# Jeffrey-Ede/AI-CV-Automation-Elect-Micr

Measured on AMD Instinct MI355X. Metric: megapixels/sec restored (512x512x1 bs=32), higher is better.
Workload: dtype bf16x3 (split-bf16 MFMA inputs, fp32 accumulate and activations)

## Files before the change

### ai-cv-automation-elect-micr_amd/_lib.py

```python
from __future__ import annotations

import ctypes as C
import os

PKG_DIR = os.path.dirname(os.path.abspath(__file__))
LIB_PATH = os.environ.get("EMD_LIB_PATH") or os.path.join(PKG_DIR, "libemdenoise.so")

EMD_OK = 0
EMD_K_SYMMETRIC = 1

_c_float_p = C.c_void_p

class PackJob(C.Structure):
    _fields_ = [("w", C.c_void_p), ("hi", C.c_void_p), ("lo", C.c_void_p), ("tap_sel", C.c_ulonglong), ("total", C.c_long),
                ("first_block", C.c_long), ("n_blocks", C.c_long), ("ntaps", C.c_int), ("cin", C.c_int), ("cout", C.c_int),
                ("cout_major", C.c_int), ("cpad", C.c_int), ("pad_", C.c_int)]


class KFusedJob(C.Structure):
    _fields_ = [("theta", C.c_void_p), ("adam_m", C.c_void_p), ("adam_v", C.c_void_p), ("step", C.c_void_p),
                ("params_out", C.c_void_p), ("losses", C.c_void_p), ("width", C.c_int), ("depth", C.c_int)]


SIGNATURES = {
# ... 188 lines not shown
    "emd_conv3x3_cout1_wgrad_f32": (C.c_int, [_c_float_p, C.c_int, _c_float_p, _c_float_p] + [C.c_int] * 4 + [C.c_void_p]),
    "emd_conv3x3_cout1_bwd_data_f32": (C.c_int, [_c_float_p, _c_float_p, _c_float_p, C.c_int] + [C.c_int] * 4 + [C.c_void_p]),
    "emd_resize_bilinear_bwd_f32": (C.c_int, [_c_float_p, C.c_int, _c_float_p, C.c_int] + [C.c_int] * 6 + [C.c_void_p]),
    "emd_avgpool2x2_bwd_f32": (C.c_int, [_c_float_p, C.c_int, _c_float_p, C.c_int] + [C.c_int] * 4 + [C.c_void_p]),
    "emd_axpy_f32": (C.c_int, [_c_float_p, C.c_int, _c_float_p, C.c_int, C.c_long, C.c_int, C.c_float, C.c_void_p]),
    "emd_denoise_loss_workspace_bytes": (C.c_size_t, []),
    "emd_denoise_loss_f32": (C.c_int, [_c_float_p, _c_float_p, C.c_long, C.c_float, _c_float_p, _c_float_p, C.c_void_p,
                                       C.c_void_p]),
    "emd_nesterov_step_f32": (C.c_int, [_c_float_p, _c_float_p, _c_float_p, C.c_long, C.c_float, C.c_float, C.c_float,
                                        C.c_void_p]),
    "emd_dw3x3_reflect_f32": (C.c_int, [_c_float_p, C.c_int, _c_float_p, _c_float_p, C.c_int] + [C.c_int] * 5 + [C.c_void_p]),
    "emd_cin1_k7_reflect_f32": (C.c_int, [_c_float_p] * 5 + [C.c_int] * 6 + [C.c_void_p]),
    "emd_conv3x3_cout1_reflect_f32": (C.c_int, [_c_float_p, C.c_int, _c_float_p, C.c_float, _c_float_p] + [C.c_int] * 4 +
                                      [C.c_void_p]),
    "emd_instnorm_tanh_f32": (C.c_int, [_c_float_p] * 4 + [C.c_int, C.c_long, C.c_float, C.c_void_p]),
    "emd_sep3x3_fused_reflect_f32": (C.c_int, [_c_float_p, C.c_int, _c_float_p, C.c_void_p, C.c_void_p, _c_float_p, _c_float_p,
                                               _c_float_p, _c_float_p, _c_float_p, C.c_int, _c_float_p, C.c_int, C.c_int,
                                               C.c_int, C.c_int, C.c_int, C.c_int, C.c_int, C.c_int, C.c_void_p]),
    "emd_dw3x3_reflect_gen_f32": (C.c_int, [_c_float_p, C.c_int, _c_float_p, _c_float_p, C.c_int, _c_float_p, _c_float_p] +
                                  [C.c_int] * 6 + [C.c_void_p]),
    "emd_sep3x3_fused_gen_f32": (C.c_int, [_c_float_p, C.c_int, _c_float_p, _c_float_p, C.c_int, _c_float_p, C.c_void_p,
                                           C.c_void_p, _c_float_p, _c_float_p, _c_float_p, _c_float_p, _c_float_p, C.c_int,
                                           _c_float_p, C.c_int] + [C.c_int] * 8 + [C.c_void_p]),
    "emd_fc_rows_f32": (C.c_int, [_c_float_p, C.c_int, _c_float_p, C.c_float, _c_float_p, C.c_int, C.c_int, C.c_void_p]),
    "emd_max3_sigmoid_f32": (C.c_int, [_c_float_p] * 4 + [C.c_int, C.c_void_p]),
    "emd_gan_head_f32": (C.c_int, [_c_float_p, C.c_float, C.c_int, C.c_float, _c_float_p, _c_float_p, C.c_void_p]),
    "emd_fc_row_bwd_f32": (C.c_int, [_c_float_p] * 6 + [C.c_int, C.c_void_p]),
    "emd_bcast_rows_f32": (C.c_int, [_c_float_p, _c_float_p, C.c_int, C.c_long, C.c_int, C.c_float, C.c_void_p]),
    "emd_sumsq_workspace_bytes": (C.c_size_t, []),
    "emd_sumsq_f32": (C.c_int, [_c_float_p, C.c_long, C.c_float, _c_float_p, C.c_void_p, C.c_void_p]),
    "emd_adam_step_f32": (C.c_int, [_c_float_p] * 4 + [C.c_long] + [C.c_float] * 5 + [_c_float_p, C.c_float, C.c_void_p]),
    "emd_dw3x3_reflect_wgrad_f32": (C.c_int, [_c_float_p, C.c_int, _c_float_p, C.c_int, _c_float_p] + [C.c_int] * 5 + [C.c_void_p]),
    "emd_dw3x3_reflect_bwd_data_f32": (C.c_int, [_c_float_p, C.c_int, _c_float_p, _c_float_p, C.c_int] + [C.c_int] * 5 + [C.c_void_p]),
    "emd_conv3x3_cout1_reflect_wgrad_f32": (C.c_int, [_c_float_p, C.c_int, _c_float_p, _c_float_p] + [C.c_int] * 4 + [C.c_void_p]),
    "emd_conv3x3_cout1_reflect_bwd_data_f32": (C.c_int, [_c_float_p, _c_float_p, _c_float_p, C.c_int] + [C.c_int] * 4 + [C.c_void_p]),
    "emd_dw7_c1_reflect_f32": (C.c_int, [_c_float_p] * 3 + [C.c_int] * 3 + [C.c_void_p]),
    "emd_dw7_c1_reflect_wgrad_f32": (C.c_int, [_c_float_p] * 3 + [C.c_int] * 3 + [C.c_void_p]),
    "emd_tanh_bwd_f32": (C.c_int, [_c_float_p] * 3 + [C.c_long, C.c_void_p]),
    "emd_l1_feature_f32": (C.c_int, [_c_float_p, _c_float_p, C.c_long, C.c_float, _c_float_p, C.c_int, _c_float_p, C.c_void_p]),
    "emd_crop_scatter_f32": (C.c_int, [_c_float_p, C.c_int, _c_float_p] + [C.c_int] * 4 + [C.c_void_p]),
    "emd_crop_scatter_dev_f32": (C.c_int, [_c_float_p, C.c_int, _c_float_p, C.c_void_p, C.c_int, C.c_int, C.c_void_p]),
    "emd_adam_step_dev_f32": (C.c_int, [_c_float_p] * 4 + [C.c_long, _c_float_p] + [C.c_float] * 4 + [_c_float_p, C.c_float, C.c_void_p]),
    "emd_bn_infer_fold2_f32": (C.c_int, [_c_float_p] * 8 + [C.c_float, C.c_int] + [_c_float_p] * 6 + [C.c_void_p]),
    "emd_bn_infer_grads_f32": (C.c_int, [_c_float_p] * 4 + [C.c_int] + [_c_float_p] * 4 + [C.c_void_p]),
    "emd_sep3x3_gemm_supported": (C.c_int, [C.c_int] * 4),
    "emd_sep3x3_gemm_f32": (C.c_int, [_c_float_p, C.c_int, _c_float_p, C.c_void_p, C.c_void_p, _c_float_p, _c_float_p, _c_float_p, _c_float_p,
# ... 177 lines not shown
```

### ai-cv-automation-elect-micr_amd/csrc/graph_exec.hip

```cpp
#include <cmath>
#include <cstdlib>
#include <cstring>
#include <map>
#include <string>
#include <vector>

#include "graph_common.hpp"

namespace {

constexpr int F0 = 64, F1 = 128, F2 = 256, F3 = 728, F4 = 728, AF = 728, AOUT = 256, NEXTRA = 11;
constexpr double BN_EPS = 1e-3;

enum Kind { SEP, CONV, DECONV, BNONLY };

struct LayerDecl {
    std::string key;
    Kind kind;
    int cin, cout, k = 1, stride = 1, rate = 1;
    std::string wname = "weights", bname = "biases";
    std::string scope;
    std::vector<std::string> bn;
    std::string extra_bn;
};
// ... 387 lines not shown
        }
        T4 cur[2] = {part(x, 0), part(x, 1)}, oh[2] = {part(out, 0), part(out, 1)};
        for (int blk = -1; blk < NEXTRA; ++blk)
            for (int h = 0; h < 2; ++h) {
                ar = &sub[h];
                st = dry ? st0 : g->side[h];
                middle_block(blk, &cur[h], &oh[h]);
            }
        ar = ar0;
        st = st0;
        if (!dry) {
            for (int h = 0; h < 2; ++h)
                if (hipEventRecord(g->join[h], g->side[h]) != hipSuccess || hipStreamWaitEvent(st0, g->join[h], 0) != hipSuccess)
                    call(emd::fail(EMD_E_LAUNCH, "emd_graph_run: stream join failed"));
        }
        for (int h = 0; h < 2; ++h) ar->release(mem[h]);
        return out;
    }

    void forward(const float* xin, float* yout, int B, int S) {
        const int S2 = S / 2, S4 = S / 4, S16 = S / 16;
        auto& P = g->P;
        T4 cnn0_last;
        if (emd_sep3x3_fused_supported(S, S, F0, F0, 1, 1)) {
            T4 d4 = E(B, S, S, 4);
            cnn0_last = E(B, S, S, F0);
            if (live()) {
                const LayerParams &pc = P["cnn0"], &pl = P["cnn0_last"];
                call(emd_cin1_f32(xin, pc.w9, g->unit4, g->zero4, d4.ptr(), d4.ld, B, S, S, 4, 1, 0, st));
                call(emd_sep3x3_fused_gen_f32(d4.ptr(), d4.ld, pc.a, pc.shift, EMD_ACT_RELU6, pl.dw, pl.pw.hi, pl.pw.lo, pl.scale, pl.shift, nullptr,
                                              nullptr, nullptr, 0, cnn0_last.ptr(), cnn0_last.ld, B, S, S, F0, F0, EMD_ACT_RELU6, EMD_PREC_BF16X3, 0, st));
            }
            free(d4);
        } else {
            T4 cnn0 = E(B, S, S, F0);
            if (live()) call(emd_cin1_f32(xin, P["cnn0"].w9, P["cnn0"].a, P["cnn0"].shift, cnn0.ptr(), cnn0.ld, B, S, S, F0, 1, 1, st));
            cnn0_last = sep("cnn0_last", cnn0, nullptr, nullptr);
            free(cnn0);
        }
        T4 concat1 = E(B, S2, S2, F2 + F1);
        T4 c1s = concat1.slice(F2, F1);
        T4 cnn0_strided;
        const LayerParams& ps = P["cnn0_strided"];
        if (ps.d.stride == 2 && ps.d.rate == 1 && emd_sep3x3_fused_supported(S, S, ps.d.cin, ps.d.cout, 2, 1) &&
            emd_sep3x3_fused_s2_genres_supported(S, S, ps.d.cin, ps.d.cout)) {
            cnn0_strided = c1s;
            if (live())
// ... 310 lines not shown
```

### ai-cv-automation-elect-micr_amd/csrc/sep_fused.hip

```cpp
#include <cstdlib>

#include "sep_params.hpp"

using namespace emd;

namespace {

__device__ __attribute__((aligned(16))) float g_zero_px[4096];

inline int sep_nt() { return (g_knobs.nt_mask >> 1) & 1; }
inline int sep_xcd() { return g_knobs.sep_xcd; }

template <int BN, int PASSES, bool GEN, int TH = 8, bool DUAL = false, bool WRES = false>
__global__ __launch_bounds__(256, 2) void sep_fused_kernel(const SepParams p) {
    constexpr int TW = 16, BM = TH * TW, BK = 32;
    constexpr int PH = TH + 2, PW = TW + 2, NPX = PH * PW;
    constexpr int PLD = 40;
    constexpr int LDK = BK + 8;
    constexpr int WN = BN / 64, WM = 4 / WN;
    constexpr int TM = BM / WM / 32, TN = BN / WN / 32;
    constexpr int NPL = PASSES == 3 ? 2 : 1;
    constexpr int P_PASSES = (NPX * 8 + 255) / 256;
    constexpr int W_PASSES = BN / 64;
    constexpr int NPT = BM / 32;
// ... 338 lines not shown
#pragma unroll 4
                for (int r = er; r < BM; r += ROWS_PER_PASS)
                    put(r, finish(*reinterpret_cast<const f32x4*>(&stage[r][ncol])));
            }
        }
        __syncthreads();
        SEP_STAMP(6)
#pragma unroll
        for (int i = 0; i < TM; ++i)
#pragma unroll
            for (int j = 0; j < TN; ++j)
#pragma unroll
                for (int e = 0; e < 16; ++e) acc[i][j][e] = 0.f;
        x0 += TW;
    }
    if (p.stamps && tid == 0) {
        long long* o = p.stamps + ((long)(blockIdx.z * gridDim.y + blockIdx.y) * gridDim.x + blockIdx.x) * 8;
#pragma unroll
        for (int i = 0; i < 8; ++i) o[i] = ph[i];
    }
#undef SEP_STAMP
}


int tiles_per_workgroup(int tiles_w, long wgs1) {
    const int force = g_knobs.sep_tpw;
    int tpw = 1;
    for (int t = 8; t >= 2; t >>= 1)
        if (tiles_w % t == 0 && wgs1 / t >= 2048) { tpw = t; break; }
    if (force > 0 && tiles_w % force == 0) tpw = force;
    return tpw;
}

int launch_wres(const SepParams& p, int B, hipStream_t st) {
    SepParams q = p;
    const int tiles_w = p.W / 16;
    q.tpw = tiles_per_workgroup(tiles_w, (long)tiles_w * (p.H / 8) * B);
    q.stamps = g_knobs.sep_stamps;
    const dim3 grid(tiles_w / q.tpw, p.H / 8, B);
    q.nt = sep_nt();
    q.xcd = sep_xcd() && ((long)grid.x * grid.y * grid.z) % 8 == 0;
    if (p.gen_a) hipLaunchKernelGGL((sep_fused_kernel<64, 3, true, 8, false, true>), grid, dim3(256), 0, st, q);
    else hipLaunchKernelGGL((sep_fused_kernel<64, 3, false, 8, false, true>), grid, dim3(256), 0, st, q);
    return emd::check_launch("sep_fused_kernel<resident W>");
}

template <int BN>
int launch(const SepParams& p, int B, int passes, hipStream_t st) {
    if constexpr (BN == 64) {
        const int wres = g_knobs.sep_wres;
        if (wres && p.Cin <= 64 && passes == 3) return launch_wres(p, B, st);
    }
    SepParams q = p;
    const int tiles_w = p.W / 16;
    q.tpw = tiles_per_workgroup(tiles_w, (long)tiles_w * (p.H / 8) * B);
    q.stamps = g_knobs.sep_stamps;
    const dim3 grid(tiles_w / q.tpw, p.H / 8, B);
    q.nt = sep_nt();
    q.xcd = sep_xcd() && ((long)grid.x * grid.y * grid.z) % 8 == 0;
    if (p.gen_a) {
        if (passes == 3)
            hipLaunchKernelGGL((sep_fused_kernel<BN, 3, true>), grid, dim3(256), 0, st, q);
        else
            hipLaunchKernelGGL((sep_fused_kernel<BN, 1, true>), grid, dim3(256), 0, st, q);
    } else if (passes == 3)
        hipLaunchKernelGGL((sep_fused_kernel<BN, 3, false>), grid, dim3(256), 0, st, q);
    else
// ... 213 lines not shown
    return sep_fused_entry(x, ldx, dw, whi, wlo, scale1, shift1, scale2, shift2, res, ldres, static_cast<float*>(y), ldy, B, H, W, Cin,
                           Cout, act, 3, 0, stream, nullptr, nullptr, 0, 1);
}

extern "C" int emd_sep3x3_fused_reflect_f32(const float* x, int ldx, const float* dw, const uint16_t* whi,
                                            const uint16_t* wlo, const float* scale1, const float* shift1,
                                            const float* scale2, const float* shift2, const float* res, int ldres,
                                            float* y, int ldy, int B, int H, int W, int Cin, int Cout, int act,
                                            int precision, emd_stream_t stream) {
    return sep_fused_entry(x, ldx, dw, whi, wlo, scale1, shift1, scale2, shift2, res, ldres, y, ldy, B, H, W, Cin, Cout, act,
                           precision, 1, stream);
}

extern "C" int emd_sep3x3_fused_gen_f32(const float* d, int ldd, const float* gen_a, const float* gen_t, int gen_act,
                                        const float* dw, const uint16_t* whi, const uint16_t* wlo, const float* scale1,
                                        const float* shift1, const float* scale2, const float* shift2, const float* res,
                                        int ldres, float* y, int ldy, int B, int H, int W, int Cin, int Cout, int act,
                                        int precision, int reflect, emd_stream_t stream) {
    EMD_REQUIRE(gen_a && gen_t, EMD_E_INVALID, "emd_sep3x3_fused_gen_f32: null gen_a / gen_t");
    return sep_fused_entry(d, ldd, dw, whi, wlo, scale1, shift1, scale2, shift2, res, ldres, y, ldy, B, H, W, Cin, Cout, act,
                           precision, reflect, stream, gen_a, gen_t, gen_act);
}

extern "C" void emd_debug_sep_stamps(void* buf) { g_knobs.sep_stamps = static_cast<long long*>(buf); }

extern "C" int emd_sep3x3_dual_supported(int H, int W, int Cin, int Cout, int Cout2) {
    const bool wide = Cout > 64 || Cout2 > 64;
    return H % (wide ? 4 : 8) == 0 && W % 16 == 0 && Cin % 32 == 0 && Cin >= 32 && Cin <= 4096 && Cout % 4 == 0 && Cout2 % 4 == 0 &&
           Cout >= 4 && Cout2 >= 4 && Cout <= 128 && Cout2 <= 128;
}

extern "C" int emd_sep3x3_dual_preferred(int H, int W, int Cin, int Cout, int Cout2) {
    if (!emd_sep3x3_dual_supported(H, W, Cin, Cout, Cout2)) return 0;
    if (Cout <= 64 && Cout2 <= 64) return 1;
    return H % 8 == 0 && W % 32 == 0;
}

extern "C" int emd_sep3x3_dual_f32(const float* x, int ldx, const float* dw, const uint16_t* whi, const uint16_t* wlo,
                                   const float* scale1, const float* shift1, float* y, int ldy, const uint16_t* w2hi,
                                   const uint16_t* w2lo, const float* scale_b, const float* shift_b, float* y2, int ldy2, int B, int H,
                                   int W, int Cin, int Cout, int Cout2, int act, emd_stream_t stream) {
    EMD_REQUIRE(x && dw && whi && wlo && scale1 && shift1 && y && w2hi && w2lo && scale_b && shift_b && y2, EMD_E_INVALID,
                "emd_sep3x3_dual_f32: null pointer");
    EMD_REQUIRE(B >= 0 && H >= 1 && W >= 1, EMD_E_INVALID, "emd_sep3x3_dual_f32: bad shape");
    EMD_REQUIRE(emd_sep3x3_dual_supported(H, W, Cin, Cout, Cout2), EMD_E_UNSUPPORTED,
                "emd_sep3x3_dual_f32: needs H%8==0 (H%4==0 above 64 output channels), W%16==0, Cin%32==0, Cout%4==0, Cout<=128 (both outputs)");
// ... 21 lines not shown
```

### ai-cv-automation-elect-micr_amd/csrc/sep_params.hpp

```cpp
#pragma once

#include "mfma_common.hpp"

namespace emd {

struct SepParams {
    const float* x;
    const float* dw;
    const uint16_t* Whi;
    const uint16_t* Wlo;
    float* y;
    const float* res;
    const float* scale1;
    const float* shift1;
    const float* scale2;
    const float* shift2;
    int H, W, Cin, Cpad, N;
    int ldx, ldy, ldres, act;
    int stride;
    int reflect;
    int tpw;
    const float* gen_a;
    const float* gen_t;
    int gen_act;
    int rg_stride;
    union { const uint16_t* W2hi; const float* rg_x; };
    union { const uint16_t* W2lo; const float* fold_w; };
    union { float* y2; float* fold_z; };
    union { const float* scale_b; const float* rg_a; };
    union { const float* shift_b; const float* rg_t; };
    int N2;
    union { int ldy2; int fold; };
    int out_split;
    int rg_ld;
    long long* stamps;
    int nt;
    int ablate;
    int xcd;
    int rg_act;
};
inline bool folded(const SepParams& p) { return p.N2 == 0 && p.fold != 0; }
static_assert(sizeof(SepParams) == 232, "SepParams: the rg_* fields fill padding and share storage; see above before adding a field");

bool sep_pipe_covers(const SepParams& p, int precision);
int sep_pipe_launch(const SepParams& p, int B, hipStream_t st);
bool sep_pipe2_covers(const SepParams& p);
int sep_pipe2_launch(const SepParams& p, int B, hipStream_t st);

}
// ... 1 lines not shown
```

### ai-cv-automation-elect-micr_amd/denoiser.py

```python
from __future__ import annotations

import os
from collections import OrderedDict

import numpy as np

from . import _lib, ops, streams

features0, features1, features2, features3, features4 = 64, 128, 256, 728, 728
aspp_filters = features4
aspp_output = 256
aspp_rateSmall, aspp_rateMedium, aspp_rateLarge = 6, 12, 18
num_extra_blocks = 11
cropsize = 512
channels = 1
BN_EPS = 1e-3

DATA_DIR = os.path.join(os.path.dirname(os.path.abspath(__file__)), "data")
SYNTH_SEED = 1234


class _Scope:

    def __init__(self):
# ... 397 lines not shown
                self._forward_pass(x[half:], out[half:], stage=lambda name: sb.wait_event(ev[name]), stage_first=True)
            main.wait_stream(sa)
            main.wait_stream(sb)
        finally:
            self.two_streams = two
        return out

    def _forward_pass(self, x, out=None, stage=None, stage_first=False):
        import torch

        B, S = x.shape[0], x.shape[1]
        assert x.shape[2] == S and S % 16 == 0 and S >= 16, "square crops with side a multiple of 16"
        dev = self.device
        if stage is not None and stage_first:
            stage("enc")
        E = lambda H, Cc: ops.Act.empty(B, H, H, Cc, dev)
        P = self.P
        S2, S4, S8, S16 = S // 2, S // 4, S // 8, S // 16
        f0, f1, f2, f3 = features0, features1, features2, features3

        if (self.fuse_sep and os.environ.get("EMD_D_GEN", "1") != "0"
                and bool(_lib.load().emd_sep3x3_fused_supported(S, S, f0, f0, 1, 1))):
            pc, pl = P["cnn0"], P["cnn0_last"]
            d4 = ops.cin1(x, pc["w9"], self._unit4, self._zero4, E(S, 4), act=False)
            cnn0 = None
            cnn0_last = ops.sep_fused_gen(d4, pc["a"], pc["shift"], pl["dw"], pl["pw"], pl["scale"], pl["shift"], E(S, f0),
                                          scale2=pl.get("scale2"), shift2=pl.get("shift2"), precision=self.precision)
        else:
            cnn0 = ops.cin1(x, P["cnn0"]["w9"], P["cnn0"]["a"], P["cnn0"]["shift"], E(S, f0))
            cnn0_last = self._sep("cnn0_last", cnn0)
        concat1 = E(S2, f2 + f1)
        if self._residual0_generated(cnn0_last):
            ps, pr = P["cnn0_strided"], P["residual0"]
            cnn0_strided = ops.sep_fused(cnn0_last, ps["dw"], ps["pw"], ps["scale"], ps["shift"], concat1.slice(f2, f1),
                                         scale2=ps.get("scale2"), shift2=ps.get("shift2"), precision=self.precision, stride=2,
                                         gen_res=(x, pr["a"], pr["shift"]))
        else:
            residual0 = ops.cin1(x, None, P["residual0"]["a"], P["residual0"]["shift"], E(S2, f1), stride=2)
            cnn0_strided = self._sep("cnn0_strided", cnn0_last, out=concat1.slice(f2, f1), res=residual0)
            del residual0
        del cnn0, cnn0_last
        residual1 = self._conv1x1("residual1", cnn0_strided)
        cnn1 = self._sep("cnn1", cnn0_strided)
        cnn1_last = self._sep("cnn1_last", cnn1)
        concat2 = E(S4, aspp_output + f1)
        cnn1_strided = self._sep("cnn1_strided", cnn1_last, out=concat2.slice(aspp_output, f1), res=residual1)
        del cnn1, cnn1_last, residual1
        residual2 = self._conv1x1("residual2", cnn1_strided)
        cnn2 = self._sep("cnn2", cnn1_strided)
        cnn2_last = self._sep("cnn2_last", cnn2)
# ... 188 lines not shown
```

### ai-cv-automation-elect-micr_amd/ops.py

```python
from __future__ import annotations

import ctypes as C

import numpy as np

from . import _lib

PREC_BF16 = 1
PREC_BF16X3 = 3
ACT_NONE, ACT_RELU6, ACT_RELU, ACT_RELU6_CLIP01, ACT_LEAKY = 0, 1, 2, 3, 4


def _act(a):
    return int(a) if not isinstance(a, bool) else (ACT_RELU6 if a else ACT_NONE)


class Act:

    __slots__ = ("buf", "B", "H", "W", "C", "ld", "c0")

    def __init__(self, buf, C_=None, c0=0):
        assert buf.dim() == 4 and buf.is_contiguous() and str(buf.dtype) == "torch.float32" and buf.is_cuda
        self.buf = buf
        self.B, self.H, self.W, self.ld = buf.shape
# ... 244 lines not shown


def sep_dual_supported(x: Act, cout: int, cout2: int) -> bool:
    return bool(_lib.load().emd_sep3x3_dual_supported(x.H, x.W, x.C, cout, cout2))


def sep_dual_preferred(x: Act, cout: int, cout2: int) -> bool:
    return bool(_lib.load().emd_sep3x3_dual_preferred(x.H, x.W, x.C, cout, cout2))


def sep_dual(x: Act, dw_dev, w: PackedWeights, w2: PackedWeights, scale1, shift1, out: Act, scale_b, shift_b, out2: Act, act=True,
             stream=None):
    lib = _lib.load()
    assert (out.B, out.H, out.W, out.C) == (x.B, x.H, x.W, w.cout) and w.cin == x.C and w.taps == 1
    assert (out2.B, out2.H, out2.W, out2.C) == (x.B, x.H, x.W, w2.cout) and w2.cin == x.C and w2.taps == 1
    rc = lib.emd_sep3x3_dual_f32(x.ptr, x.ld, _p(dw_dev), _p(w.hi), _p(w.lo), _p(scale1), _p(shift1), out.ptr, out.ld, _p(w2.hi), _p(w2.lo),
                                 _p(scale_b), _p(shift_b), out2.ptr, out2.ld, x.B, x.H, x.W, x.C, w.cout, w2.cout, _act(act),
                                 _lib.stream_ptr(stream))
    _lib.check(rc, "emd_sep3x3_dual_f32")
    return out, out2


def sep_fused_gen(d: Act, gen_a, gen_t, dw_dev, w: PackedWeights, scale1, shift1, out: Act, gen_act=True, act=True,
                  scale2=None, shift2=None, res: Act | None = None, precision=PREC_BF16X3, stream=None, reflect=False):
    lib = _lib.load()
    assert (out.B, out.H, out.W, out.C) == (d.B, d.H, d.W, w.cout) and w.taps == 1
    assert gen_a.numel() == w.cin and gen_t.numel() == w.cin
    if res is not None:
        assert (res.B, res.H, res.W, res.C) == (out.B, out.H, out.W, out.C)
    rc = lib.emd_sep3x3_fused_gen_f32(d.ptr, d.ld, _p(gen_a), _p(gen_t), _act(gen_act), _p(dw_dev), _p(w.hi), _p(w.lo),
                                      _p(scale1), _p(shift1), _p(scale2), _p(shift2),
                                      res.ptr if res is not None else C.c_void_p(0), res.ld if res is not None else 0,
                                      out.ptr, out.ld, d.B, d.H, d.W, w.cin, w.cout, _act(act), precision,
                                      1 if reflect else 0, _lib.stream_ptr(stream))
    _lib.check(rc, "emd_sep3x3_fused_gen_f32")
    return out


def deconv3x3s2(x: Act, w_phases, scale1, shift1, out: Act, act=True, precision=PREC_BF16X3, stream=None):
    lib = _lib.load()
    assert len(w_phases) == 4 and (out.B, out.H, out.W) == (x.B, 2 * x.H, 2 * x.W) and out.C == w_phases[0].cout
    hi = (C.c_void_p * 4)(*[w.hi.data_ptr() for w in w_phases])
    lo = (C.c_void_p * 4)(*[w.lo.data_ptr() for w in w_phases])
    rc = lib.emd_deconv3x3s2_f32(x.ptr, x.ld, hi, lo, _p(scale1), _p(shift1), out.ptr, out.ld, x.B, x.H, x.W, x.C,
                                 out.C, _act(act), precision, _lib.stream_ptr(stream))
    _lib.check(rc, "emd_deconv3x3s2_f32")
    return out


def deconv_phase_taps(phase):
    lib = _lib.load()
    ky = (C.c_int * 4)()
# ... 360 lines not shown
```

### include/emdenoise.h

```cpp
#ifndef EMDENOISE_H
#define EMDENOISE_H

#include <stddef.h>
#include <stdint.h>

#ifdef __cplusplus
extern "C" {
#endif

#define EMD_VERSION 100

#define EMD_OK 0
#define EMD_E_INVALID (-1)
#define EMD_E_UNSUPPORTED (-2)
#define EMD_E_ALIGN (-3)
#define EMD_E_LAUNCH (-4)
#define EMD_E_ALLOC (-5)

typedef void* emd_stream_t;

int emd_version(void);
const char* emd_last_error(void);

#define EMD_K_MAX_WIDTH 15
// ... 348 lines not shown
                        const float* scale1, const float* shift1, float* y, int ldy, const uint16_t* w2hi,
                        const uint16_t* w2lo, const float* scale_b, const float* shift_b, float* y2, int ldy2, int B, int H,
                        int W, int Cin, int Cout, int Cout2, int act, emd_stream_t stream);

int emd_sep3x3_gemm_supported(int H, int W, int Cin, int Cout);
int emd_sep3x3_gemm_f32(const float* x, int ldx, const float* dw, const uint16_t* whi, const uint16_t* wlo,
                        const float* scale1, const float* shift1, const float* scale2, const float* shift2,
                        const float* res, int ldres, float* y, int ldy, int B, int H, int W, int Cin, int Cout, int act,
                        emd_stream_t stream);

int emd_sep3x3_fused_reflect_f32(const float* x, int ldx, const float* dw, const uint16_t* whi, const uint16_t* wlo,
                                 const float* scale1, const float* shift1, const float* scale2, const float* shift2,
                                 const float* res, int ldres, float* y, int ldy, int B, int H, int W, int Cin, int Cout,
                                 int act, int precision, emd_stream_t stream);

int emd_dw3x3_reflect_gen_f32(const float* d, int ldd, const float* gen_a, const float* gen_t, int leaky_act, const float* w,
                              float* y, int ldy, int B, int H, int W, int C, int stride, emd_stream_t stream);

int emd_sep3x3_fused_gen_f32(const float* d, int ldd, const float* gen_a, const float* gen_t, int gen_act, const float* dw,
                             const uint16_t* whi, const uint16_t* wlo, const float* scale1, const float* shift1,
                             const float* scale2, const float* shift2, const float* res, int ldres, float* y, int ldy, int B,
                             int H, int W, int Cin, int Cout, int act, int precision, int reflect, emd_stream_t stream);

int emd_fc_rows_f32(const float* x, int ldx, const float* w, float bias, float* y, int B, int K, emd_stream_t stream);
int emd_max3_sigmoid_f32(const float* a, const float* b, const float* c, float* y, int n, emd_stream_t stream);


int emd_gan_head_f32(const float* logit3, float label, int mode, float grad_scale, float* result2, float* dlogit3,
                     emd_stream_t stream);
int emd_fc_row_bwd_f32(const float* x, const float* w, const float* dlogit, float* dw, float* db, float* dx, int K,
                       emd_stream_t stream);
int emd_bcast_rows_f32(const float* v, float* y, int ldy, long npix, int C, float alpha, emd_stream_t stream);
size_t emd_sumsq_workspace_bytes(void);
int emd_sumsq_f32(const float* x, long n, float scale, float* out, void* workspace, emd_stream_t stream);
int emd_adam_step_f32(float* param, const float* grad, float* m, float* v, long n, float lr_t, float beta1, float beta2,
                      float eps, float grad_scale, const float* gnorm_sq, float clip_norm, emd_stream_t stream);
int emd_adam_step_dev_f32(float* param, const float* grad, float* m, float* v, long n, const float* lr_t_dev, float beta1,
                          float beta2, float eps, float grad_scale, const float* gnorm_sq, float clip_norm,
                          emd_stream_t stream);

int emd_dw3x3_reflect_wgrad_f32(const float* x, int ldx, const float* dy, int ldd, float* dw, int B, int H, int W, int C,
                                int stride, emd_stream_t stream);
int emd_dw3x3_reflect_bwd_data_f32(const float* dy, int ldd, const float* w, float* dx, int ldx, int B, int H, int W, int C,
                                   int stride, emd_stream_t stream);
int emd_conv3x3_cout1_reflect_wgrad_f32(const float* x, int ldx, const float* dy, float* dw, int B, int H, int W, int Cin,
                                        emd_stream_t stream);
// ... 173 lines not shown
```

Baseline: 385.0.

## Fuse the 3x3 cin=1 stem conv into the fused separable conv kernel

```diff
diff --git a/ai-cv-automation-elect-micr_amd/_lib.py b/ai-cv-automation-elect-micr_amd/_lib.py
--- a/ai-cv-automation-elect-micr_amd/_lib.py
+++ b/ai-cv-automation-elect-micr_amd/_lib.py
@@ -234,6 +234,10 @@
     "emd_sep3x3_fused_gen_f32": (C.c_int, [_c_float_p, C.c_int, _c_float_p, _c_float_p, C.c_int, _c_float_p, C.c_void_p,
                                            C.c_void_p, _c_float_p, _c_float_p, _c_float_p, _c_float_p, _c_float_p, C.c_int,
                                            _c_float_p, C.c_int] + [C.c_int] * 8 + [C.c_void_p]),
+    "emd_sep3x3_fused_gen9_supported": (C.c_int, [C.c_int] * 4),
+    "emd_sep3x3_fused_gen9_f32": (C.c_int, [_c_float_p, _c_float_p, _c_float_p, _c_float_p, C.c_int, _c_float_p, C.c_void_p,
+                                            C.c_void_p, _c_float_p, _c_float_p, _c_float_p, _c_float_p, _c_float_p, C.c_int,
+                                            _c_float_p, C.c_int] + [C.c_int] * 8 + [C.c_void_p]),
     "emd_fc_rows_f32": (C.c_int, [_c_float_p, C.c_int, _c_float_p, C.c_float, _c_float_p, C.c_int, C.c_int, C.c_void_p]),
     "emd_max3_sigmoid_f32": (C.c_int, [_c_float_p] * 4 + [C.c_int, C.c_void_p]),
     "emd_gan_head_f32": (C.c_int, [_c_float_p, C.c_float, C.c_int, C.c_float, _c_float_p, _c_float_p, C.c_void_p]),
diff --git a/ai-cv-automation-elect-micr_amd/csrc/graph_exec.hip b/ai-cv-automation-elect-micr_amd/csrc/graph_exec.hip
--- a/ai-cv-automation-elect-micr_amd/csrc/graph_exec.hip
+++ b/ai-cv-automation-elect-micr_amd/csrc/graph_exec.hip
@@ -433,7 +433,14 @@
         const int S2 = S / 2, S4 = S / 4, S16 = S / 16;
         auto& P = g->P;
         T4 cnn0_last;
-        if (emd_sep3x3_fused_supported(S, S, F0, F0, 1, 1)) {
+        if (emd_sep3x3_fused_gen9_supported(S, S, F0, F0)) {
+            cnn0_last = E(B, S, S, F0);
+            if (live()) {
+                const LayerParams &pc = P["cnn0"], &pl = P["cnn0_last"];
+                call(emd_sep3x3_fused_gen9_f32(xin, pc.w9, pc.a, pc.shift, EMD_ACT_RELU6, pl.dw, pl.pw.hi, pl.pw.lo, pl.scale, pl.shift, nullptr,
+                                               nullptr, nullptr, 0, cnn0_last.ptr(), cnn0_last.ld, B, S, S, F0, F0, EMD_ACT_RELU6, EMD_PREC_BF16X3, 0, st));
+            }
+        } else if (emd_sep3x3_fused_supported(S, S, F0, F0, 1, 1)) {
             T4 d4 = E(B, S, S, 4);
             cnn0_last = E(B, S, S, F0);
             if (live()) {
diff --git a/ai-cv-automation-elect-micr_amd/csrc/sep_fused.hip b/ai-cv-automation-elect-micr_amd/csrc/sep_fused.hip
--- a/ai-cv-automation-elect-micr_amd/csrc/sep_fused.hip
+++ b/ai-cv-automation-elect-micr_amd/csrc/sep_fused.hip
@@ -1,4 +1,5 @@
 #include <cstdlib>
+#include <type_traits>
 
 #include "sep_params.hpp"
 
@@ -384,6 +385,247 @@
 #undef SEP_STAMP
 }
 
+template <int NCH, bool RES>
+__global__ __launch_bounds__(256, 2) void sep_gen9_kernel(const SepParams p) {
+    constexpr int TH = 8, TW = 16, BM = TH * TW, BN = 64, BK = 32, LDK = BK + 8;
+    constexpr int DH = TH + 2, DW = TW + 2, DLD = 20, ND = DH * DW;
+    constexpr int LDS_STAGE = BN + 4;
+    constexpr int B_CHUNK = 2 * BN * LDK * 2, A_CHUNK = 2 * BM * LDK * 2;
+    constexpr int D_BYTES = DH * DLD * 4, STAGE_BYTES = BM * LDS_STAGE * 4;
+    constexpr int D_OFF = NCH * B_CHUNK, A_OFF = D_OFF + 2 * D_BYTES;
+    constexpr int TILE_BYTES = A_OFF + (NCH * A_CHUNK > STAGE_BYTES ? NCH * A_CHUNK : STAGE_BYTES);
+    static_assert(A_OFF % 16 == 0 && (DLD * 4) % 16 == 0, "16-byte reads of the d tile and the A planes");
+
+    __shared__ __attribute__((aligned(16))) unsigned char smem[TILE_BYTES];
+    float* dt = reinterpret_cast<float*>(smem + D_OFF);
+    float(*stage)[LDS_STAGE] = reinterpret_cast<float(*)[LDS_STAGE]>(smem + A_OFF);
+
+    const int tid = threadIdx.x;
+    const int lane = tid & 63;
+    const int wv = tid >> 6;
+    int bx = blockIdx.x, by = blockIdx.y, bz = blockIdx.z;
+    xcd_remap(p.xcd, bx, by, bz);
+    const int xbase = bx * p.tpw * TW, y0 = by * TH;
+    const long img = (long)bz * p.H * p.W;
+
+    {
+        const int w_col = (tid & 3) * 8, w_row = tid >> 2;
+        const uint16_t* __restrict__ whi = p.Whi + (long)w_row * p.Cpad + w_col;
+        const uint16_t* __restrict__ wlo = p.Wlo + (long)w_row * p.Cpad + w_col;
+#pragma unroll
+        for (int c = 0; c < NCH; ++c) {
+            auto Bc = reinterpret_cast<uint16_t(*)[BN][LDK]>(smem + c * B_CHUNK);
+            *reinterpret_cast<u32x4*>(&Bc[0][w_row][w_col]) = *reinterpret_cast<const u32x4*>(whi + c * BK);
+            *reinterpret_cast<u32x4*>(&Bc[1][w_row][w_col]) = *reinterpret_cast<const u32x4*>(wlo + c * BK);
+        }
+    }
+    const int c4 = tid & 7, pg = tid >> 3;
+    const int ty = pg >> 2, tx0 = (pg & 3) * 4;
+    f32x4 wk[NCH][9], ga[NCH], gt[NCH];
+#pragma unroll
+    for (int c = 0; c < NCH; ++c) {
+#pragma unroll
+        for (int k = 0; k < 9; ++k) wk[c][k] = *reinterpret_cast<const f32x4*>(p.dw + (long)k * p.Cin + c * BK + c4 * 4);
+        ga[c] = *reinterpret_cast<const f32x4*>(p.gen_a + c * BK + c4 * 4);
+        gt[c] = *reinterpret_cast<const f32x4*>(p.gen_t + c * BK + c4 * 4);
+    }
+    const int di = tid < ND ? tid : ND - 1;
+    const int dpy = di / DW, dpx = di - dpy * DW;
+    bool rok[3];
+    const float* irow[3];
+#pragma unroll
+    for (int i = 0; i < 3; ++i) {
+        const int ry = y0 - 2 + dpy + i;
+        rok[i] = ry >= 0 && ry < p.H;
+        irow[i] = p.x + img + (long)(ry < 0 ? 0 : (ry >= p.H ? p.H - 1 : ry)) * p.W;
+    }
+    float w9[9];
+#pragma unroll
+    for (int k = 0; k < 9; ++k) w9[k] = p.gen_w9[k];
+    float iv[9];
+    auto load_img = [&](int xt) {
+#pragma unroll
+        for (int j = 0; j < 3; ++j) {
+            const int rx = xt - 2 + dpx + j;
+            const int cx = rx < 0 ? 0 : (rx >= p.W ? p.W - 1 : rx);
+#pragma unroll
+            for (int i = 0; i < 3; ++i) iv[i * 3 + j] = irow[i][cx];
+        }
+    };
+    auto form_d = [&](int xt, int buf) {
+        float d = 0.f;
+#pragma unroll
+        for (int i = 0; i < 3; ++i)
+#pragma unroll
+            for (int j = 0; j < 3; ++j) {
+                const int rx = xt - 2 + dpx + j;
+                d = (rok[i] && rx >= 0 && rx < p.W) ? fmaf(w9[i * 3 + j], iv[i * 3 + j], d) : d;
+            }
+        if (tid < ND) dt[buf * (DH * DLD) + dpy * DLD + dpx] = d;
+    };
+
+    f32x16 acc[2];
+#pragma unroll
+    for (int j = 0; j < 2; ++j)
+#pragma unroll
+        for (int e = 0; e < 16; ++e) acc[j][e] = 0.f;
+    const int fr = lane & 31, fh = lane >> 5;
+    constexpr int E_C4 = BN / 4, E_RPP = 256 / E_C4, E_NROWS = BM / E_RPP;
+    const int ncol = (tid % E_C4) * 4, er = tid / E_C4;
+
+    load_img(xbase);
+    form_d(xbase, 0);
+#pragma unroll
+    for (int c = 0; c < NCH; ++c) {
+#pragma unroll
+        for (int k = 0; k < 9; ++k) asm volatile("" : "+v"(wk[c][k]));
+        asm volatile("" : "+v"(ga[c]), "+v"(gt[c]));
+    }
+    __syncthreads();
+
+    for (int t = 0; t < p.tpw; ++t) {
+        const int x0 = xbase + t * TW;
+        float dv[3][6];
+        {
+            const float* dsrc = dt + (t & 1) * (DH * DLD) + ty * DLD + tx0;
+#pragma unroll
+            for (int i = 0; i < 3; ++i) {
+                const f32x4 q = *reinterpret_cast<const f32x4*>(dsrc + i * DLD);
+                const f32x2 r = *reinterpret_cast<const f32x2*>(dsrc + i * DLD + 4);
+                dv[i][0] = q[0]; dv[i][1] = q[1]; dv[i][2] = q[2]; dv[i][3] = q[3]; dv[i][4] = r[0]; dv[i][5] = r[1];
+            }
+        }
+        const bool more = t + 1 < p.tpw;
+        if (more) load_img(x0 + TW);
+        auto stage1 = [&](auto border) {
+            constexpr bool BORDER = decltype(border)::value;
+            bool rowok[3];
+#pragma unroll
+            for (int i = 0; i < 3; ++i) rowok[i] = y0 - 1 + ty + i >= 0 && y0 - 1 + ty + i < p.H;
+            const bool c0ok = x0 - 1 + tx0 >= 0, c5ok = x0 + tx0 + 4 < p.W;
+#pragma unroll
+            for (int c = 0; c < NCH; ++c) {
+                f32x4 o[4];
+#pragma unroll
+                for (int j = 0; j < 4; ++j) o[j] = f32x4{0.f, 0.f, 0.f, 0.f};
+#pragma unroll
+                for (int i = 0; i < 3; ++i) {
+                    f32x4 pr[6];
+#pragma unroll
+                    for (int d = 0; d < 6; ++d) {
+                        const float dd = dv[i][d];
+                        const f32x4 u = __builtin_elementwise_fma(f32x4{dd, dd, dd, dd}, ga[c], gt[c]);
+#pragma unroll
+                        for (int ch = 0; ch < 4; ++ch) pr[d][ch] = __builtin_amdgcn_fmed3f(u[ch], 0.f, 6.f);
+                        if (BORDER) {
+                            const bool ok = rowok[i] && (d == 0 ? c0ok : (d == 5 ? c5ok : true));
+                            if (!ok) pr[d] = f32x4{0.f, 0.f, 0.f, 0.f};
+                        }
+                    }
+#pragma unroll
+                    for (int j = 0; j < 4; ++j)
+#pragma unroll
+                        for (int d = 0; d < 3; ++d) o[j] += wk[c][i * 3 + d] * pr[j + d];
+                }
+                auto Ac = reinterpret_cast<uint16_t(*)[BM][LDK]>(smem + A_OFF + c * A_CHUNK);
+#pragma unroll
+                for (int j = 0; j < 4; ++j) {
+                    const int r = ty * TW + tx0 + j;
+                    unsigned h0, l0, h1, l1;
+                    split2(o[j][0], o[j][1], h0, l0);
+                    split2(o[j][2], o[j][3], h1, l1);
+                    *reinterpret_cast<u32x2*>(&Ac[0][r][c4 * 4]) = u32x2{h0, h1};
+                    *reinterpret_cast<u32x2*>(&Ac[1][r][c4 * 4]) = u32x2{l0, l1};
+                }
+            }
+        };
+        if (y0 == 0 || y0 + TH == p.H || x0 == 0 || x0 + TW == p.W) stage1(std::true_type{});
+        else stage1(std::false_type{});
+        const int ncl = ncol < p.N ? ncol : 0;
+        f32x4 rve[RES ? E_NROWS : 1];
+        if constexpr (RES) {
+            const float* __restrict__ rt = p.res + (img + (long)y0 * p.W) * p.ldres + ncl;
+#pragma unroll
+            for (int k = 0; k < E_NROWS; ++k) {
+                const int r = er + k * E_RPP;
+                rve[k] = *reinterpret_cast<const f32x4*>(rt + ((r >> 4) * p.W + (r & 15) + x0) * p.ldres);
+            }
+        }
+        const bool two = p.scale2 != nullptr;
+        f32x4 s1 = *reinterpret_cast<const f32x4*>(p.scale1 + ncl);
+        f32x4 t1 = *reinterpret_cast<const f32x4*>(p.shift1 + ncl);
+        f32x4 s2 = *reinterpret_cast<const f32x4*>((two ? p.scale2 : p.scale1) + ncl);
+        f32x4 t2 = *reinterpret_cast<const f32x4*>((two ? p.shift2 : p.shift1) + ncl);
+        __syncthreads();
+#pragma unroll
+        for (int c = 0; c < NCH; ++c) {
+            auto Ac = reinterpret_cast<const uint16_t(*)[BM][LDK]>(smem + A_OFF + c * A_CHUNK);
+            auto Bc = reinterpret_cast<const uint16_t(*)[BN][LDK]>(smem + c * B_CHUNK);
+#pragma unroll
+            for (int ks = 0; ks < BK / 16; ++ks) {
+                const int r = wv * 32 + fr;
+                const bf16x8 ah = *reinterpret_cast<const bf16x8*>(&Ac[0][r][ks * 16 + fh * 8]);
+                const bf16x8 al = *reinterpret_cast<const bf16x8*>(&Ac[1][r][ks * 16 + fh * 8]);
+                bf16x8 bh[2], bl[2];
+#pragma unroll
+                for (int j = 0; j < 2; ++j) {
+                    bh[j] = *reinterpret_cast<const bf16x8*>(&Bc[0][j * 32 + fr][ks * 16 + fh * 8]);
+                    bl[j] = *reinterpret_cast<const bf16x8*>(&Bc[1][j * 32 + fr][ks * 16 + fh * 8]);
+                }
+#pragma unroll
+                for (int j = 0; j < 2; ++j) {
+                    acc[j] = __builtin_amdgcn_mfma_f32_32x32x16_bf16(al, bh[j], acc[j], 0, 0, 0);
+                    acc[j] = __builtin_amdgcn_mfma_f32_32x32x16_bf16(ah, bl[j], acc[j], 0, 0, 0);
+                    acc[j] = __builtin_amdgcn_mfma_f32_32x32x16_bf16(ah, bh[j], acc[j], 0, 0, 0);
+                }
+            }
+        }
+        if (more) form_d(x0 + TW, (t + 1) & 1);
+        __syncthreads();
+
+#pragma unroll
+        for (int j = 0; j < 2; ++j)
+#pragma unroll
+            for (int e = 0; e < 16; ++e) {
+                const int r = wv * 32 + (e & 3) + 8 * (e >> 2) + 4 * fh;
+                stage[r][j * 32 + fr] = acc[j][e];
+                acc[j][e] = 0.f;
+            }
+        __syncthreads();
+        asm volatile("" : "+v"(s1), "+v"(t1), "+v"(s2), "+v"(t2));
+        if constexpr (RES) {
+#pragma unroll
+            for (int k = 0; k < E_NROWS; ++k) asm volatile("" : "+v"(rve[k]));
+        }
+        if (ncol < p.N) {
+            const float hi = p.act == 1 ? 6.f : __builtin_inff();
+            const float hi2 = p.act == 2 ? __builtin_inff() : 6.f;
+            const float slope = p.act == 4 ? 0.2f : 1.f, lo = (p.act == 1 || p.act == 2) ? 0.f : -__builtin_inff();
+            auto finish = [&](f32x4 v) {
+#pragma unroll
+                for (int c = 0; c < 4; ++c) {
+                    float u = fmaf(v[c], s1[c], t1[c]);
+                    u = fminf(fmaxf(fmaxf(u, lo), slope * u), hi);
+                    if (two) u = fminf(fmaxf(fmaf(u, s2[c], t2[c]), 0.f), hi2);
+                    v[c] = u;
+                }
+                return v;
+            };
+            float* __restrict__ ytile = p.y + (img + (long)y0 * p.W) * p.ldy + ncl;
+#pragma unroll
+            for (int k = 0; k < E_NROWS; ++k) {
+                const int r = er + k * E_RPP;
+                f32x4 v = finish(*reinterpret_cast<const f32x4*>(&stage[r][ncl]));
+                if constexpr (RES) v = v + rve[k];
+                float* dst = ytile + ((r >> 4) * p.W + (r & 15) + x0) * p.ldy;
+                if (p.nt) store_nt16(dst, v);
+                else *reinterpret_cast<f32x4*>(dst) = v;
+            }
+        }
+        __syncthreads();
+    }
+}
+
 
 int tiles_per_workgroup(int tiles_w, long wgs1) {
     const int force = g_knobs.sep_tpw;
@@ -405,6 +647,24 @@
     if (p.gen_a) hipLaunchKernelGGL((sep_fused_kernel<64, 3, true, 8, false, true>), grid, dim3(256), 0, st, q);
     else hipLaunchKernelGGL((sep_fused_kernel<64, 3, false, 8, false, true>), grid, dim3(256), 0, st, q);
     return emd::check_launch("sep_fused_kernel<resident W>");
+}
+
+int launch_gen9(const SepParams& p, int B, hipStream_t st) {
+    SepParams q = p;
+    const int tiles_w = p.W / 16;
+    q.tpw = tiles_per_workgroup(tiles_w, (long)tiles_w * (p.H / 8) * B);
+    const dim3 grid(tiles_w / q.tpw, p.H / 8, B);
+    q.nt = sep_nt();
+    q.xcd = sep_xcd() && ((long)grid.x * grid.y * grid.z) % 8 == 0;
+    if (p.Cin == 64) {
+        if (p.res) hipLaunchKernelGGL((sep_gen9_kernel<2, true>), grid, dim3(256), 0, st, q);
+        else hipLaunchKernelGGL((sep_gen9_kernel<2, false>), grid, dim3(256), 0, st, q);
+    } else if (p.res) {
+        hipLaunchKernelGGL((sep_gen9_kernel<1, true>), grid, dim3(256), 0, st, q);
+    } else {
+        hipLaunchKernelGGL((sep_gen9_kernel<1, false>), grid, dim3(256), 0, st, q);
+    }
+    return emd::check_launch("sep_gen9_kernel");
 }
 
 template <int BN>
@@ -664,6 +924,42 @@
                            precision, reflect, stream, gen_a, gen_t, gen_act);
 }
 
+extern "C" int emd_sep3x3_fused_gen9_supported(int H, int W, int Cin, int Cout) {
+    return H >= 8 && W >= 16 && H % 8 == 0 && W % 16 == 0 && (Cin == 32 || Cin == 64) && Cout % 4 == 0 && Cout >= 4 && Cout <= 64;
+}
+
+extern "C" int emd_sep3x3_fused_gen9_f32(const float* img, const float* w9, const float* gen_a, const float* gen_t, int gen_act,
+                                         const float* dw, const uint16_t* whi, const uint16_t* wlo, const float* scale1,
+                                         const float* shift1, const float* scale2, const float* shift2, const float* res,
+                                         int ldres, float* y, int ldy, int B, int H, int W, int Cin, int Cout, int act,
+                                         int precision, int reflect, emd_stream_t stream) {
+    EMD_REQUIRE(img && w9 && gen_a && gen_t && dw && whi && wlo && scale1 && shift1 && y, EMD_E_INVALID,
+                "emd_sep3x3_fused_gen9_f32: null pointer");
+    EMD_REQUIRE((scale2 == nullptr) == (shift2 == nullptr), EMD_E_INVALID, "emd_sep3x3_fused_gen9_f32: scale2/shift2 pair");
+    EMD_REQUIRE(B >= 0 && H >= 1 && W >= 1, EMD_E_INVALID, "emd_sep3x3_fused_gen9_f32: bad shape");
+    EMD_REQUIRE(gen_act == EMD_ACT_RELU6 && !reflect && precision == 3 && emd_sep3x3_fused_gen9_supported(H, W, Cin, Cout),
+                EMD_E_UNSUPPORTED,
+                "emd_sep3x3_fused_gen9_f32: needs relu6 generation, zero padding, split-bf16, H%8==0, W%16==0, Cin 32 or 64, Cout%4==0, "
+                "Cout<=64 (use emd_cin1_f32 + emd_sep3x3_fused_gen_f32)");
+    EMD_REQUIRE(B <= 65535, EMD_E_UNSUPPORTED, "emd_sep3x3_fused_gen9_f32: B > 65535");
+    EMD_REQUIRE(9L * W * (ldy > ldres ? ldy : ldres) < (1L << 31), EMD_E_UNSUPPORTED,
+                "emd_sep3x3_fused_gen9_f32: 9 image rows of the output must span fewer than 2^31 floats");
+    EMD_REQUIRE(ldy % 4 == 0 && ldy >= Cout && (!res || (ldres % 4 == 0 && ldres >= Cout)), EMD_E_ALIGN,
+                "emd_sep3x3_fused_gen9_f32: pixel strides must be multiples of 4 and >= the channel count");
+    EMD_REQUIRE(emd::aligned16(gen_a) && emd::aligned16(gen_t) && emd::aligned16(dw) && emd::aligned16(whi) && emd::aligned16(wlo) &&
+                    emd::aligned16(y) && (!res || emd::aligned16(res)) && emd::aligned16(scale1) && emd::aligned16(shift1) &&
+                    (!scale2 || (emd::aligned16(scale2) && emd::aligned16(shift2))),
+                EMD_E_ALIGN, "emd_sep3x3_fused_gen9_f32: pointers (but img, w9) must be 16-byte aligned");
+    if (B == 0) return EMD_OK;
+    SepParams p{};
+    p.x = img; p.dw = dw; p.Whi = whi; p.Wlo = wlo; p.y = y; p.res = res;
+    p.scale1 = scale1; p.shift1 = shift1; p.scale2 = scale2; p.shift2 = shift2;
+    p.H = H; p.W = W; p.Cin = Cin; p.Cpad = (Cin + kBK - 1) / kBK * kBK; p.N = Cout;
+    p.ldx = 1; p.ldy = ldy; p.ldres = ldres; p.act = act; p.stride = 1;
+    p.gen_a = gen_a; p.gen_t = gen_t; p.gen_act = gen_act; p.gen_w9 = w9;
+    return launch_gen9(p, B, static_cast<hipStream_t>(stream));
+}
+
 extern "C" void emd_debug_sep_stamps(void* buf) { g_knobs.sep_stamps = static_cast<long long*>(buf); }
 
 extern "C" int emd_sep3x3_dual_supported(int H, int W, int Cin, int Cout, int Cout2) {
diff --git a/ai-cv-automation-elect-micr_amd/csrc/sep_params.hpp b/ai-cv-automation-elect-micr_amd/csrc/sep_params.hpp
--- a/ai-cv-automation-elect-micr_amd/csrc/sep_params.hpp
+++ b/ai-cv-automation-elect-micr_amd/csrc/sep_params.hpp
@@ -24,7 +24,7 @@
     const float* gen_t;
     int gen_act;
     int rg_stride;
-    union { const uint16_t* W2hi; const float* rg_x; };
+    union { const uint16_t* W2hi; const float* rg_x; const float* gen_w9; };
     union { const uint16_t* W2lo; const float* fold_w; };
     union { float* y2; float* fold_z; };
     union { const float* scale_b; const float* rg_a; };
diff --git a/ai-cv-automation-elect-micr_amd/denoiser.py b/ai-cv-automation-elect-micr_amd/denoiser.py
--- a/ai-cv-automation-elect-micr_amd/denoiser.py
+++ b/ai-cv-automation-elect-micr_amd/denoiser.py
@@ -443,10 +443,16 @@
         if (self.fuse_sep and os.environ.get("EMD_D_GEN", "1") != "0"
                 and bool(_lib.load().emd_sep3x3_fused_supported(S, S, f0, f0, 1, 1))):
             pc, pl = P["cnn0"], P["cnn0_last"]
-            d4 = ops.cin1(x, pc["w9"], self._unit4, self._zero4, E(S, 4), act=False)
             cnn0 = None
-            cnn0_last = ops.sep_fused_gen(d4, pc["a"], pc["shift"], pl["dw"], pl["pw"], pl["scale"], pl["shift"], E(S, f0),
-                                          scale2=pl.get("scale2"), shift2=pl.get("shift2"), precision=self.precision)
+            if (self.precision == ops.PREC_BF16X3 and os.environ.get("EMD_D_GEN9", "1") != "0"
+                    and bool(_lib.load().emd_sep3x3_fused_gen9_supported(S, S, f0, f0))):
+                cnn0_last = ops.sep_fused_gen(ops.Act(x), pc["a"], pc["shift"], pl["dw"], pl["pw"], pl["scale"], pl["shift"], E(S, f0),
+                                              scale2=pl.get("scale2"), shift2=pl.get("shift2"), precision=self.precision,
+                                              gen_w9=pc["w9"])
+            else:
+                d4 = ops.cin1(x, pc["w9"], self._unit4, self._zero4, E(S, 4), act=False)
+                cnn0_last = ops.sep_fused_gen(d4, pc["a"], pc["shift"], pl["dw"], pl["pw"], pl["scale"], pl["shift"], E(S, f0),
+                                              scale2=pl.get("scale2"), shift2=pl.get("shift2"), precision=self.precision)
         else:
             cnn0 = ops.cin1(x, P["cnn0"]["w9"], P["cnn0"]["a"], P["cnn0"]["shift"], E(S, f0))
             cnn0_last = self._sep("cnn0_last", cnn0)
diff --git a/ai-cv-automation-elect-micr_amd/ops.py b/ai-cv-automation-elect-micr_amd/ops.py
--- a/ai-cv-automation-elect-micr_amd/ops.py
+++ b/ai-cv-automation-elect-micr_amd/ops.py
@@ -290,12 +290,21 @@
 
 
 def sep_fused_gen(d: Act, gen_a, gen_t, dw_dev, w: PackedWeights, scale1, shift1, out: Act, gen_act=True, act=True,
-                  scale2=None, shift2=None, res: Act | None = None, precision=PREC_BF16X3, stream=None, reflect=False):
+                  scale2=None, shift2=None, res: Act | None = None, precision=PREC_BF16X3, stream=None, reflect=False, gen_w9=None):
     lib = _lib.load()
     assert (out.B, out.H, out.W, out.C) == (d.B, d.H, d.W, w.cout) and w.taps == 1
     assert gen_a.numel() == w.cin and gen_t.numel() == w.cin
     if res is not None:
         assert (res.B, res.H, res.W, res.C) == (out.B, out.H, out.W, out.C)
+    if gen_w9 is not None:
+        assert d.C == 1 and d.ld == 1 and gen_w9.numel() == 9
+        rc = lib.emd_sep3x3_fused_gen9_f32(d.ptr, _p(gen_w9), _p(gen_a), _p(gen_t), _act(gen_act), _p(dw_dev), _p(w.hi), _p(w.lo),
+                                           _p(scale1), _p(shift1), _p(scale2), _p(shift2),
+                                           res.ptr if res is not None else C.c_void_p(0), res.ld if res is not None else 0,
+                                           out.ptr, out.ld, d.B, d.H, d.W, w.cin, w.cout, _act(act), precision,
+                                           1 if reflect else 0, _lib.stream_ptr(stream))
+        _lib.check(rc, "emd_sep3x3_fused_gen9_f32")
+        return out
     rc = lib.emd_sep3x3_fused_gen_f32(d.ptr, d.ld, _p(gen_a), _p(gen_t), _act(gen_act), _p(dw_dev), _p(w.hi), _p(w.lo),
                                       _p(scale1), _p(shift1), _p(scale2), _p(shift2),
                                       res.ptr if res is not None else C.c_void_p(0), res.ld if res is not None else 0,
diff --git a/include/emdenoise.h b/include/emdenoise.h
--- a/include/emdenoise.h
+++ b/include/emdenoise.h
@@ -394,6 +394,12 @@
                              const float* scale2, const float* shift2, const float* res, int ldres, float* y, int ldy, int B,
                              int H, int W, int Cin, int Cout, int act, int precision, int reflect, emd_stream_t stream);
 
+int emd_sep3x3_fused_gen9_supported(int H, int W, int Cin, int Cout);
+int emd_sep3x3_fused_gen9_f32(const float* img, const float* w9, const float* gen_a, const float* gen_t, int gen_act, const float* dw,
+                              const uint16_t* whi, const uint16_t* wlo, const float* scale1, const float* shift1,
+                              const float* scale2, const float* shift2, const float* res, int ldres, float* y, int ldy, int B,
+                              int H, int W, int Cin, int Cout, int act, int precision, int reflect, emd_stream_t stream);
+
 int emd_fc_rows_f32(const float* x, int ldx, const float* w, float bias, float* y, int B, int K, emd_stream_t stream);
 int emd_max3_sigmoid_f32(const float* a, const float* b, const float* c, float* y, int n, emd_stream_t stream);
 
```

New measurement: 390.0, median of 6. 1.01x the previous value.
